# cure-lab/MagicDrive

Measured on NVIDIA H100. Metric: 6-view 224x400 denoising-steps/sec, higher is better.
Workload: dtype bf16

## Files before the change

include/magicdrive_b200.h:

```cpp
#ifndef MAGICDRIVE_B200_H
#define MAGICDRIVE_B200_H

#include <stddef.h>
#include <stdint.h>

#ifdef __cplusplus
extern "C" {
#endif

#define MDB_OK 0
#define MDB_ERR_INVALID (-1)
#define MDB_ERR_CUDA (-2)
#define MDB_ERR_UNSUPPORTED (-3)

const char* mdb_last_error(void);

int mdb_set_pdl(int on);
int mdb_version(void);
int mdb_device_ok(void);

typedef struct {
  const void* a0;
  const void* a1;
  int c0, lda0, c1, lda1;
  int n_img, h_in, w_in;
  const void* w;
  int n_out;
  int taps_h, taps_w, stride, pad_h, pad_w;
  int h_out, w_out;
  const float* bias;
  const float* rowbias;
  int rowbias_ld;
  const void* residual;
  int ldr;
  void* out;
  int ldo;
  int out_is_f32;
  float out_scale;
  int epi_mode;
  void* workspace;
  size_t workspace_bytes;
  int force_block_n;
  int force_splits;
  int kernel_variant;
  const float* ln_stats;
  int ln_parts;
  float ln_eps;
  const float* ln_colsum;
  float* stats_out;
} mdb_gemm_desc;

int mdb_gemm_conv(const mdb_gemm_desc* d, void* stream);
int mdb_gemm_conv_launches(const mdb_gemm_desc* d);
int mdb_gemm_conv_stats_parts(const mdb_gemm_desc* d);

int mdb_conv_direct(const void* x, int x_is_f32, int n, int h, int w, int cin, const float* wgt, const float* bias,
                    int cout, int kh, int kw, int stride_h, int stride_w, int pad_h, int pad_w, int ho, int wo,
                    int silu, const void* residual, void* out, int out_is_f32, void* stream);

int mdb_groupnorm(const void* x0, int c0, int ld0, const void* x1, int c1, int ld1, int n_img, int hw, int groups,
                  float eps, const float* gamma, const float* beta, int silu, void* out, int ldo, float* stats_ws,
                  void* stream);

int mdb_layernorm(const void* x, long long rows, int c, int ldx, const float* gamma, const float* beta, float eps,
                  void* out, int ldo, void* stream);

int mdb_softmax_rows(const float* s, int lds, long long rows, int cols, void* out, int ldo, int cols_out, void* stream);

int mdb_attention(const void* q, int ldq, const void* k, int ldk, const void* v, int ldv, void* out, int ldo, int b,
                  int b_kv, int heads, int lq, int lk, int d, const int* kv_index, int n_sets, float scale, void* stream);

int mdb_attention_multi(const void* q, int ldq, int n_src, const void* const* k, const int* ldk, const void* const* v,
                        const int* ldv, const int* b_kv, void* out, int ldo, int b, int heads, int lq, int lk, int d,
                        const int* kv_index, int n_sets, float scale, void* stream);

int mdb_add(const void* a, const void* b, void* out, long long n, void* stream);

int mdb_upsample_nearest(const void* x, int n, int h, int w, int c, void* out, int ho, int wo, void* stream);
int mdb_adaptive_avgpool(const float* x, int n, int h, int w, int c, float* out, int ho, int wo, int silu, void* stream);

int mdb_linear_small(const float* in, int m, int k, int ldi, const void* w, int ldw, const float* bias, int n,
                     int pre_silu, int post_silu, float* out, int ldo, void* stream);

int mdb_timestep_embedding(const float* t, int m, int dim, int flip_sin_to_cos, float freq_shift, float* out,
                           void* stream);

int mdb_fourier_embed(const float* x, long long rows, int d, int num_freqs, float* out, void* stream);
// ... 30 lines not shown
```

magicdrive_b200/_lib.py:

```python
import ctypes as C
import os
from pathlib import Path

_LIB = None
LIB_PATH = Path(os.environ.get("MDB_LIB_PATH") or Path(__file__).resolve().parent / "lib" / "libmagicdrive_b200.so")


class MdbError(RuntimeError):
    pass


class GemmDesc(C.Structure):
    _fields_ = [
        ("a0", C.c_void_p), ("a1", C.c_void_p),
        ("c0", C.c_int), ("lda0", C.c_int), ("c1", C.c_int), ("lda1", C.c_int),
        ("n_img", C.c_int), ("h_in", C.c_int), ("w_in", C.c_int),
        ("w", C.c_void_p), ("n_out", C.c_int),
        ("taps_h", C.c_int), ("taps_w", C.c_int), ("stride", C.c_int), ("pad_h", C.c_int), ("pad_w", C.c_int),
        ("h_out", C.c_int), ("w_out", C.c_int),
        ("bias", C.c_void_p), ("rowbias", C.c_void_p), ("rowbias_ld", C.c_int),
        ("residual", C.c_void_p), ("ldr", C.c_int),
        ("out", C.c_void_p), ("ldo", C.c_int), ("out_is_f32", C.c_int), ("out_scale", C.c_float),
        ("epi_mode", C.c_int),
        ("workspace", C.c_void_p), ("workspace_bytes", C.c_size_t),
        ("force_block_n", C.c_int), ("force_splits", C.c_int), ("kernel_variant", C.c_int),
        ("ln_stats", C.c_void_p), ("ln_parts", C.c_int), ("ln_eps", C.c_float), ("ln_colsum", C.c_void_p),
        ("stats_out", C.c_void_p),
    ]


_vp, _i, _f, _ll = C.c_void_p, C.c_int, C.c_float, C.c_longlong
SIGNATURES = {
    "mdb_last_error": (C.c_char_p, []),
    "mdb_set_pdl": (_i, [_i]),
    "mdb_version": (_i, []),
    "mdb_device_ok": (_i, []),
    "mdb_gemm_conv": (_i, [C.POINTER(GemmDesc), _vp]),
    "mdb_gemm_conv_launches": (_i, [C.POINTER(GemmDesc)]),
    "mdb_gemm_conv_stats_parts": (_i, [C.POINTER(GemmDesc)]),
    "mdb_conv_direct": (_i, [_vp, _i, _i, _i, _i, _i, _vp, _vp, _i, _i, _i, _i, _i, _i, _i, _i, _i, _i, _vp, _vp, _i, _vp]),
    "mdb_groupnorm": (_i, [_vp, _i, _i, _vp, _i, _i, _i, _i, _i, _f, _vp, _vp, _i, _vp, _i, _vp, _vp]),
    "mdb_layernorm": (_i, [_vp, _ll, _i, _i, _vp, _vp, _f, _vp, _i, _vp]),
    "mdb_attention": (_i, [_vp, _i, _vp, _i, _vp, _i, _vp, _i, _i, _i, _i, _i, _i, _i, _vp, _i, _f, _vp]),
    "mdb_attention_multi": (_i, [_vp, _i, _i, _vp, _vp, _vp, _vp, _vp, _vp, _i, _i, _i, _i, _i, _i, _vp, _i, _f, _vp]),
    "mdb_add": (_i, [_vp, _vp, _vp, _ll, _vp]),
    "mdb_upsample_nearest": (_i, [_vp, _i, _i, _i, _i, _vp, _i, _i, _vp]),
    "mdb_adaptive_avgpool": (_i, [_vp, _i, _i, _i, _i, _vp, _i, _i, _i, _vp]),
    "mdb_linear_small": (_i, [_vp, _i, _i, _i, _vp, _i, _vp, _i, _i, _i, _vp, _i, _vp]),
    "mdb_timestep_embedding": (_i, [_vp, _i, _i, _i, _f, _vp, _vp]),
    "mdb_fourier_embed": (_i, [_vp, _ll, _i, _i, _vp, _vp]),
    "mdb_nchw_to_nhwc": (_i, [_vp, _i, _i, _i, _i, _i, _vp, _vp]),
    "mdb_nhwc_to_nchw": (_i, [_vp, _i, _i, _i, _i, _vp, _i, _vp]),
    "mdb_f32_to_bf16": (_i, [_vp, _vp, _ll, _vp]),
    "mdb_bf16_to_f32": (_i, [_vp, _vp, _ll, _vp]),
    "mdb_pack_latents": (_i, [_vp, _i, _ll, _i, _i, _i, _vp, _vp]),
    "mdb_cfg_ddim_step": (_i, [_vp, _i, _i, _i, _f, _vp, _vp, _ll, _vp]),
    "mdb_softmax_rows": (_i, [_vp, _i, _ll, _i, _vp, _i, _i, _vp]),
    "mdb_pin_views": (_i, [_vp, _i, _vp, _vp, _i, _vp, _vp, _ll, _i, _vp]),
    "mdb_peer_barrier": (_i, [_vp, _i, _i, _i, _i, _vp, _ll, _vp, _vp]),
    "mdb_prepare_boxes": (_i, [_vp, _i, _vp, _vp, _i, _vp, _vp, _i, _i, _vp, _vp, _vp, _vp, _vp]),
    "mdb_camera_param": (_i, [_vp, _vp, _i, _vp, _vp]),
    "mdb_cfg_unipc_step": (_i, [_vp, _i, _i, _i, _f, _vp, _vp, _vp, _vp, _vp, _ll, _vp]),
}


def lib():
    global _LIB
    if _LIB is None:
        if not LIB_PATH.exists():
            raise MdbError(
                f"{LIB_PATH} is missing: build it with `python -m magicdrive_b200.build` "
                "(there is no CPU / torch fallback for this path)")
# ... 14 lines not shown
```

magicdrive_b200/csrc/capi_gemm.cu:

```cuda
#include <cuda.h>
#include <cuda_runtime.h>
#include <stdio.h>
#include <string.h>

#include <algorithm>
#include <mutex>

#include "../../include/magicdrive_b200.h"
#define MDB_NEED_TENSORMAP
#include "common_host.h"
#include "gemm_wgmma.cuh"

using namespace mdb;

namespace {

bool make_act_map(CUtensorMap* m, const void* ptr, int c, int ld, int n, int h, int w, int bn, int bh, int bw,
                  int stride) {
  EncodeTiledFn enc = get_encode();
  if (!enc) return false;
  cuuint64_t dims[4] = {(cuuint64_t)c, (cuuint64_t)w, (cuuint64_t)h, (cuuint64_t)n};
  cuuint64_t strides[3] = {(cuuint64_t)ld * 2, (cuuint64_t)w * ld * 2, (cuuint64_t)h * w * ld * 2};
  cuuint32_t box[4] = {64u, (cuuint32_t)(bw * stride), (cuuint32_t)(bh * stride), (cuuint32_t)bn};
  cuuint32_t estr[4] = {1u, (cuuint32_t)stride, (cuuint32_t)stride, 1u};
  CUresult r = enc(m, CU_TENSOR_MAP_DATA_TYPE_BFLOAT16, 4, const_cast<void*>(ptr), dims, strides, box, estr,
                   CU_TENSOR_MAP_INTERLEAVE_NONE, CU_TENSOR_MAP_SWIZZLE_128B, CU_TENSOR_MAP_L2_PROMOTION_L2_256B,
                   CU_TENSOR_MAP_FLOAT_OOB_FILL_NONE);
  return r == CUDA_SUCCESS;
}

bool make_w_map(CUtensorMap* m, const void* ptr, int n_out, int k, int block_n) {
  EncodeTiledFn enc = get_encode();
  if (!enc) return false;
  cuuint64_t dims[2] = {(cuuint64_t)k, (cuuint64_t)n_out};
  cuuint64_t strides[1] = {(cuuint64_t)k * 2};
  cuuint32_t box[2] = {64u, (cuuint32_t)block_n};
  cuuint32_t estr[2] = {1u, 1u};
  CUresult r = enc(m, CU_TENSOR_MAP_DATA_TYPE_BFLOAT16, 2, const_cast<void*>(ptr), dims, strides, box, estr,
                   CU_TENSOR_MAP_INTERLEAVE_NONE, CU_TENSOR_MAP_SWIZZLE_128B, CU_TENSOR_MAP_L2_PROMOTION_L2_256B,
                   CU_TENSOR_MAP_FLOAT_OOB_FILL_NONE);
  return r == CUDA_SUCCESS;
}

struct Plan {
  int bn, bh, bw, tiles_n, tiles_h, tiles_w;
  int ctas, m_groups;
  int block_n, n_tiles, splits, kb_per_split, kb_total;
};

int num_sms() {
  static int sms = 0;
  if (!sms) {
    int dev = 0;
    cudaGetDevice(&dev);
    if (cudaDeviceGetAttribute(&sms, cudaDevAttrMultiProcessorCount, dev) != cudaSuccess || sms <= 0) sms = 132;
  }
  return sms;
}

void choose_box(int n_img, int h, int w, Plan* pl) {
  if (h * w <= 128) {
    int bn = 128 / (h * w);
    if (bn > n_img) bn = n_img;
    if (bn < 1) bn = 1;
    pl->bn = bn, pl->bh = h, pl->bw = w;
  } else {
    double best = -1.0;
    int bbh = 1, bbw = 1;
    const int wmax = w < 128 ? w : 128;
    for (int bw = 1; bw <= wmax; ++bw) {
      int bh = 128 / bw;
      if (bh > h) bh = h;
      if (bh < 1) continue;
      const long long tiles = (long long)((h + bh - 1) / bh) * ((w + bw - 1) / bw);
      const double eff = (double)h * w / (double)(tiles * 128);
      if (eff > best + 1e-9 || (eff > best - 1e-9 && bw > bbw)) best = eff, bbh = bh, bbw = bw;
    }
    pl->bn = 1, pl->bh = bbh, pl->bw = bbw;
  }
  pl->tiles_n = (n_img + pl->bn - 1) / pl->bn;
  pl->tiles_h = (h + pl->bh - 1) / pl->bh;
  pl->tiles_w = (w + pl->bw - 1) / pl->bw;
}

int validate(const mdb_gemm_desc* d) {
  if (!d || !d->a0 || !d->w || !d->out) return set_error(MDB_ERR_INVALID, "mdb_gemm_conv: null pointer");
  if (d->c0 <= 0 || d->c0 % 64 || d->c1 < 0 || d->c1 % 64)
    return set_error(MDB_ERR_UNSUPPORTED, "mdb_gemm_conv: channel counts must be multiples of 64 (c0=%d c1=%d)", d->c0,
                     d->c1);
  if (d->c1 > 0 && !d->a1) return set_error(MDB_ERR_INVALID, "mdb_gemm_conv: c1>0 but a1 is null");
  if (d->lda0 % 8 || (d->c1 > 0 && d->lda1 % 8) || d->ldo % 8 || (d->residual && d->ldr % 8))
    return set_error(MDB_ERR_UNSUPPORTED, "mdb_gemm_conv: leading dimensions must be multiples of 8");
  if (d->n_out % 8) return set_error(MDB_ERR_UNSUPPORTED, "mdb_gemm_conv: n_out must be a multiple of 8");
  if (d->stride != 1 && d->stride != 2) return set_error(MDB_ERR_UNSUPPORTED, "mdb_gemm_conv: stride must be 1 or 2");
  if (d->kernel_variant != 0 && (d->kernel_variant < 2 || d->kernel_variant > 4))
    return set_error(MDB_ERR_INVALID, "mdb_gemm_conv: kernel_variant must be 0, 2, 3 or 4");
  if (d->n_img <= 0 || d->h_out <= 0 || d->w_out <= 0 || d->taps_h <= 0 || d->taps_w <= 0)
    return set_error(MDB_ERR_INVALID, "mdb_gemm_conv: bad shape");
  if ((reinterpret_cast<uintptr_t>(d->a0) | reinterpret_cast<uintptr_t>(d->a1) | reinterpret_cast<uintptr_t>(d->w) |
       reinterpret_cast<uintptr_t>(d->out) | reinterpret_cast<uintptr_t>(d->residual)) & 15)
    return set_error(MDB_ERR_INVALID, "mdb_gemm_conv: pointers must be 16-byte aligned");
  if (d->epi_mode == 1 && (d->n_out % 256 || d->residual || d->rowbias || d->out_is_f32 || d->stats_out))
    return set_error(MDB_ERR_UNSUPPORTED, "mdb_gemm_conv: GEGLU epilogue needs n_out %% 256 == 0 and a plain bf16 output "
                                          "(no residual, per-image shift or row statistics)");
  return MDB_OK;
}

void plan_for(const mdb_gemm_desc* d, int ctas, bool allow_split, Plan* pl) {
  choose_box(d->n_img, d->h_out, d->w_out, pl);
  const int m_tiles = pl->tiles_n * pl->tiles_h * pl->tiles_w;
  pl->ctas = ctas;
  pl->m_groups = (m_tiles + ctas - 1) / ctas;
  pl->kb_total = d->taps_h * d->taps_w * ((d->c0 + d->c1) / 64);
  const int sms = num_sms();
  const int clusters = sms / ctas;
  int bn_choice = 0;
  if (d->epi_mode == 1) {
    bn_choice = 256;
  } else if (d->force_block_n) {
    bn_choice = d->force_block_n;
  } else {
    const int cands[4] = {256, 160, 128, 64};
    double best = 1e30;
    for (int i = 0; i < 4; ++i) {
      const int bn = cands[i];
      if (bn == 64 && d->n_out >= 128) continue;
      const int nt = (d->n_out + bn - 1) / bn;
      const long long groups = (long long)pl->m_groups * nt;
      const long long waves = (groups + clusters - 1) / clusters;
      const double cost = (double)waves * (bn < 96 ? 96 : bn) * 1.0 + (double)waves * 6.0;
      if (cost < best - 1e-9) best = cost, bn_choice = bn;
    }
  }
  pl->block_n = bn_choice;
  pl->n_tiles = (d->n_out + bn_choice - 1) / bn_choice;
  int splits = 1;
  const long long ctas_total = (long long)m_tiles * pl->n_tiles;
  if (!allow_split) {
    splits = 1;
  } else if (d->force_splits > 0) {
    splits = d->force_splits;
  } else if (d->epi_mode == 0 && !d->ln_stats && !d->stats_out && d->workspace && ctas_total * 2 <= sms && pl->kb_total >= 16) {
    splits = (int)(sms / ctas_total);
// ... 42 lines not shown
  if (e == cudaSuccess) e = cudaGetLastError();
  if (e != cudaSuccess) return set_error(MDB_ERR_CUDA, "gemm_wgmma_kernel<%d,%d> launch: %s", BN, CTAS, cudaGetErrorString(e));
  return MDB_OK;
}

template <int CTAS>
int launch_bn(int block_n, const CUtensorMap& tA0, const CUtensorMap& tA1, const CUtensorMap& tB, const GemmParams& gp,
              cudaStream_t st) {
  switch (block_n) {
    case 256: return launch<256, CTAS>(tA0, tA1, tB, gp, st);
    case 160: return launch<160, CTAS>(tA0, tA1, tB, gp, st);
    case 128: return launch<128, CTAS>(tA0, tA1, tB, gp, st);
    case 64: return launch<64, CTAS>(tA0, tA1, tB, gp, st);
    default: return set_error(MDB_ERR_UNSUPPORTED, "mdb_gemm_conv: unsupported block_n %d", block_n);
  }
}

}

extern "C" int mdb_gemm_conv_launches(const mdb_gemm_desc* d) {
  if (validate(d) != MDB_OK) return MDB_ERR_INVALID;
  Plan pl;
  make_plan(d, &pl);
  return pl.splits > 1 ? 2 : 1;
}

extern "C" int mdb_gemm_conv_stats_parts(const mdb_gemm_desc* d) {
  if (validate(d) != MDB_OK) return MDB_ERR_INVALID;
  Plan pl;
  make_plan(d, &pl);
  return pl.n_tiles;
}

extern "C" int mdb_gemm_conv(const mdb_gemm_desc* d, void* stream) {
  int rc = validate(d);
  if (rc != MDB_OK) return rc;
  if (d->ln_stats && (d->taps_h != 1 || d->taps_w != 1 || !d->ln_colsum || d->ln_parts <= 0))
    return set_error(MDB_ERR_INVALID, "mdb_gemm_conv: a folded LayerNorm needs a 1x1 GEMM, ln_colsum and ln_parts");
  Plan pl;
  make_plan(d, &pl);
  if (d->epi_mode == 1 && pl.block_n != 256) return set_error(MDB_ERR_UNSUPPORTED, "GEGLU needs block_n 256");
  cudaStream_t st = static_cast<cudaStream_t>(stream);

  CUtensorMap tA0, tA1, tB;
  if (!make_act_map(&tA0, d->a0, d->c0, d->lda0, d->n_img, d->h_in, d->w_in, pl.bn, pl.bh, pl.bw, d->stride))
    return set_error(MDB_ERR_CUDA, "cuTensorMapEncodeTiled(A0) failed (c=%d ld=%d n=%d h=%d w=%d box=%dx%dx%d s=%d)",
                     d->c0, d->lda0, d->n_img, d->h_in, d->w_in, pl.bn, pl.bh, pl.bw, d->stride);
  if (d->c1 > 0) {
    if (!make_act_map(&tA1, d->a1, d->c1, d->lda1, d->n_img, d->h_in, d->w_in, pl.bn, pl.bh, pl.bw, d->stride))
      return set_error(MDB_ERR_CUDA, "cuTensorMapEncodeTiled(A1) failed");
  } else {
    tA1 = tA0;
  }
  const int ktot = d->taps_h * d->taps_w * (d->c0 + d->c1);
  if (!make_w_map(&tB, d->w, d->n_out, ktot, pl.block_n / pl.ctas))
    return set_error(MDB_ERR_CUDA, "cuTensorMapEncodeTiled(W) failed (n=%d k=%d)", d->n_out, ktot);

  GemmParams gp;
  memset(&gp, 0, sizeof(gp));
  gp.n_img = d->n_img, gp.h_out = d->h_out, gp.w_out = d->w_out, gp.n_out = d->n_out;
  gp.taps_h = d->taps_h, gp.taps_w = d->taps_w, gp.stride = d->stride, gp.pad_h = d->pad_h, gp.pad_w = d->pad_w;
  gp.cblocks0 = d->c0 / 64, gp.cblocks1 = d->c1 / 64;
  gp.bn = pl.bn, gp.bh = pl.bh, gp.bw = pl.bw, gp.tiles_h = pl.tiles_h, gp.tiles_w = pl.tiles_w;
  gp.m_tiles = pl.tiles_n * pl.tiles_h * pl.tiles_w, gp.n_tiles = pl.n_tiles, gp.splits = pl.splits;
  gp.m_groups = pl.m_groups;
  gp.kb_per_split = pl.kb_per_split;
  gp.epi_mode = pl.splits > 1 ? EPI_PARTIAL_F32 : d->epi_mode;
  gp.out_is_f32 = d->out_is_f32;
  gp.bias = d->bias, gp.rowbias = d->rowbias, gp.rowbias_ld = d->rowbias_ld;
  gp.residual = static_cast<const __nv_bfloat16*>(d->residual), gp.ldr = d->ldr;
  gp.out = d->out, gp.ldo = d->ldo, gp.out_scale = d->out_scale;
  gp.partial = static_cast<float*>(d->workspace);
  gp.ln_stats = d->ln_stats, gp.ln_parts = d->ln_parts, gp.ln_eps = d->ln_eps, gp.ln_colsum = d->ln_colsum;
  gp.ln_inv_c = 1.0f / (float)(d->c0 + d->c1);
  gp.stats_out = d->stats_out;

  rc = pl.ctas == 2 ? launch_bn<2>(pl.block_n, tA0, tA1, tB, gp, st) : launch_bn<1>(pl.block_n, tA0, tA1, tB, gp, st);
  if (rc != MDB_OK) return rc;
  if (pl.splits > 1) {
    const long long pixels = (long long)d->n_img * d->h_out * d->w_out;
    const long long total4 = pixels * d->n_out / 4;
    const int threads = 256;
    const int blocks = (int)((total4 + threads - 1) / threads);
    cudaError_t e = launch_pdl(splitk_finalize_kernel, dim3(blocks), dim3(threads), 0, st,
                               static_cast<const float*>(d->workspace), pl.splits, pixels, d->n_out, d->h_out * d->w_out,
                               d->bias, d->rowbias, d->rowbias_ld, static_cast<const __nv_bfloat16*>(d->residual), d->ldr,
                               d->out, d->ldo, d->out_is_f32, d->out_scale);
    if (e == cudaSuccess) e = cudaGetLastError();
    if (e != cudaSuccess) return set_error(MDB_ERR_CUDA, "splitk_finalize launch: %s", cudaGetErrorString(e));
  }
  return MDB_OK;
}
```

magicdrive_b200/csrc/common_host.h:

```cpp
#pragma once
#include <stdarg.h>
#include <stdio.h>

namespace mdb {
char* error_buffer();
inline int set_error(int code, const char* fmt, ...) {
  va_list ap;
  va_start(ap, fmt);
  vsnprintf(error_buffer(), 512, fmt, ap);
  va_end(ap);
  return code;
}
}

#ifdef MDB_NEED_TENSORMAP
#include <cuda.h>
#include <cuda_runtime.h>

#include <mutex>
namespace mdb {
typedef CUresult (*EncodeTiledFn)(CUtensorMap*, CUtensorMapDataType, cuuint32_t, void*, const cuuint64_t*,
                                  const cuuint64_t*, const cuuint32_t*, const cuuint32_t*, CUtensorMapInterleave,
                                  CUtensorMapSwizzle, CUtensorMapL2promotion, CUtensorMapFloatOOBfill);
inline EncodeTiledFn get_encode() {
  static EncodeTiledFn fn = nullptr;
  static std::once_flag once;
  std::call_once(once, [] {
    void* p = nullptr;
    cudaDriverEntryPointQueryResult qres;
    if (cudaGetDriverEntryPoint("cuTensorMapEncodeTiled", &p, cudaEnableDefault, &qres) == cudaSuccess &&
        qres == cudaDriverEntryPointSuccess)
      fn = reinterpret_cast<EncodeTiledFn>(p);
  });
  return fn;
}
}
#endif

#ifdef __CUDACC__
#include <cuda_runtime.h>
#include <stdlib.h>
namespace mdb {
inline int& pdl_region_flag() {
  static int v = 0;
  return v;
}
inline bool pdl_enabled() {
  static int forced = -2;
  if (forced == -2) {
    const char* e = getenv("MDB_PDL");
    forced = e ? ((e[0] == '1') ? 1 : 0) : -1;
  }
  return forced >= 0 ? forced == 1 : pdl_region_flag() == 1;
}
inline void add_pdl_attr(cudaLaunchConfig_t& cfg, cudaLaunchAttribute* attrs, unsigned n_attrs) {
  if (pdl_enabled()) {
    attrs[n_attrs].id = cudaLaunchAttributeProgrammaticStreamSerialization;
    attrs[n_attrs].val.programmaticStreamSerializationAllowed = 1;
    ++n_attrs;
  }
  cfg.attrs = attrs;
  cfg.numAttrs = n_attrs;
}
template <typename... KArgs, typename... Args>
inline cudaError_t launch_pdl(void (*kernel)(KArgs...), dim3 grid, dim3 block, size_t smem, cudaStream_t st, Args... args) {
// ... 23 lines not shown
```

magicdrive_b200/csrc/gemm_tc.cuh:

```cuda
#pragma once
#include "ptx.cuh"

namespace mdb {

enum EpiMode : int { EPI_LINEAR = 0, EPI_GEGLU = 1, EPI_PARTIAL_F32 = 2 };

struct GemmParams {
  int n_img, h_out, w_out;
  int n_out;
  int taps_h, taps_w, stride, pad_h, pad_w;
  int cblocks0, cblocks1;
  int bn, bh, bw;
  int tiles_h, tiles_w;
  int m_tiles, n_tiles, splits;
  int m_groups;
  int kb_per_split;
  int epi_mode;
  int out_is_f32;
  const float* bias;
  const float* rowbias;
  int rowbias_ld;
  const __nv_bfloat16* residual;
  int ldr;
  void* out;
  int ldo;
  float out_scale;
  float* partial;
  const float* ln_stats;
  int ln_parts;
  float ln_inv_c, ln_eps;
  const float* ln_colsum;
  float* stats_out;
};

constexpr int kBlockM = 128;
constexpr int kBlockK = 64;
constexpr int kABytes = kBlockM * kBlockK * 2;

__device__ __forceinline__ float gelu_erf(float x) {
  const float ax = fabsf(x) * 0.70710678118654752440f;
  float t, e;
  asm("rcp.approx.ftz.f32 %0, %1;" : "=f"(t) : "f"(fmaf(0.3275911f, ax, 1.0f)));
  float poly = fmaf(t, 1.061405429f, -1.453152027f);
  poly = fmaf(poly, t, 1.421413741f);
  poly = fmaf(poly, t, -0.284496736f);
  poly = fmaf(poly, t, 0.254829592f);
// ... 42 lines not shown
```

magicdrive_b200/csrc/gemm_wgmma.cuh:

```cuda
#pragma once
#include "common_host.h"
#include "gemm_tc.cuh"
#include "ptx_cluster.cuh"
#include "wgmma.cuh"

namespace mdb {

template <int BLOCK_N, int CTAS>
struct WgGemmCfg {
  static constexpr int kBBytes = BLOCK_N * kBlockK * 2;
  static constexpr int kBRows = BLOCK_N / CTAS;
  static constexpr int kBPartBytes = kBRows * kBlockK * 2;
  static constexpr int kStageBytes = kABytes + kBBytes;
  static constexpr int kBarBytes = 256;
  static constexpr int kStagesFit = (232448 - 1024 - kBarBytes) / kStageBytes;
  static constexpr int kStages = kStagesFit > 8 ? 8 : kStagesFit;
  static constexpr int kSmemBytes = kStages * kStageBytes + 1024 + kBarBytes;
  static constexpr int kConsumerWarps = 8;
  static constexpr int kThreads = 32 * kConsumerWarps + 32;
  static constexpr int kAcc = BLOCK_N / 2;
  static_assert(kStages >= 3, "pipeline too shallow");
  static_assert(kBPartBytes % 1024 == 0, "B stage parts must keep the 1024-byte swizzle alignment");
};

// ... 7 lines not shown
  constexpr bool PAIR = CTAS == 2;
  constexpr int STAGES = Cfg::kStages;
  extern __shared__ uint8_t smem_raw[];
  uint8_t* smem = reinterpret_cast<uint8_t*>((reinterpret_cast<uintptr_t>(smem_raw) + 1023) & ~uintptr_t(1023));
  uint8_t* smA = smem;
  uint8_t* smB = smem + STAGES * kABytes;
  uint64_t* full_bar = reinterpret_cast<uint64_t*>(smem + STAGES * Cfg::kStageBytes);
  uint64_t* empty_bar = full_bar + STAGES;

  const int warp = threadIdx.x >> 5;
  const int lane = threadIdx.x & 31;
  const int cb_total = p.cblocks0 + p.cblocks1;
  const int kb_total = p.taps_h * p.taps_w * cb_total;
  const int total_tiles = p.m_groups * p.n_tiles * p.splits;
  const int rank = PAIR ? static_cast<int>(cluster_ctarank()) : 0;
  const int first_tile = static_cast<int>(blockIdx.x) / CTAS, tile_step = static_cast<int>(gridDim.x) / CTAS;

  if (warp == Cfg::kConsumerWarps && lane == 0) {
    prefetch_tmap(&tmA0);
    prefetch_tmap(&tmA1);
    prefetch_tmap(&tmB);
    for (int i = 0; i < STAGES; ++i) {
      mbar_init(&full_bar[i], 1);
      mbar_init(&empty_bar[i], CTAS * Cfg::kConsumerWarps);
    }
    fence_barrier_init();
  }
  if constexpr (PAIR) cluster_sync_all(); else __syncthreads();
  pdl_wait();
  pdl_launch_dependents();

  if (warp == Cfg::kConsumerWarps) {
    if (lane == 0) {
      const uint32_t tx_bytes = static_cast<uint32_t>(p.bn * p.bh * p.bw) * (kBlockK * 2) + Cfg::kBBytes;
      int stage = 0;
      uint32_t phase = 0;
      for (int t = first_tile; t < total_tiles; t += tile_step) {
        const int mt = (t % p.m_groups) * CTAS + rank;
        const int rest = t / p.m_groups;
        const int nt = rest % p.n_tiles;
        const int z = rest / p.n_tiles;
        const int tw = mt % p.tiles_w;
        const int th = (mt / p.tiles_w) % p.tiles_h;
        const int tn = mt / (p.tiles_w * p.tiles_h);
        const int img0 = tn * p.bn, h0 = th * p.bh, w0 = tw * p.bw;
        const int n0 = nt * BLOCK_N;
        const int kb_begin = z * p.kb_per_split;
        const int kb_end = min(kb_total, kb_begin + p.kb_per_split);
        for (int kb = kb_begin; kb < kb_end; ++kb) {
          mbar_wait(&empty_bar[stage], phase ^ 1);
          const int tap = kb / cb_total;
          const int cb = kb - tap * cb_total;
          const int r = tap / p.taps_w, s = tap - r * p.taps_w;
          mbar_arrive_expect_tx(&full_bar[stage], tx_bytes);
          const int wc = w0 * p.stride + s - p.pad_w;
          const int hc = h0 * p.stride + r - p.pad_h;
          if (cb < p.cblocks0)
            tma_load_4d(&tmA0, &full_bar[stage], smA + stage * kABytes, cb * kBlockK, wc, hc, img0);
          else
            tma_load_4d(&tmA1, &full_bar[stage], smA + stage * kABytes, (cb - p.cblocks0) * kBlockK, wc, hc, img0);
          if constexpr (PAIR)
            tma_load_2d_multicast(&tmB, &full_bar[stage], smB + stage * Cfg::kBBytes + rank * Cfg::kBPartBytes, kb * kBlockK,
                                  n0 + rank * Cfg::kBRows, 0x3);
          else
            tma_load_2d(&tmB, &full_bar[stage], smB + stage * Cfg::kBBytes, kb * kBlockK, n0);
          if (++stage == STAGES) {
            stage = 0;
            phase ^= 1;
          }
        }
      }
    }
  } else {
  const int wg = warp >> 2;
  const int q = lane & 3;
  const int row0 = 64 * wg + 16 * (warp & 3) + (lane >> 2);
  const int box_hw = p.bh * p.bw;
  int li[2], lh[2], lw[2];
#pragma unroll
  for (int h = 0; h < 2; ++h) {
    const int row = row0 + 8 * h;
    li[h] = row / box_hw;
    const int rem = row - li[h] * box_hw;
    lh[h] = rem / p.bw;
    lw[h] = rem - lh[h] * p.bw;
  }
  const long long pixels_total = static_cast<long long>(p.n_img) * p.h_out * p.w_out;
  const float scale = p.out_scale;
  int stage = 0;
  uint32_t phase = 0;
  const uint32_t peer = rank ^ 1;
  auto release = [&](int s) {
    if (lane == 0) {
      mbar_arrive(&empty_bar[s]);
      if constexpr (PAIR) mbar_arrive_cluster_release(mapa_u32(smem_u32(&empty_bar[s]), peer));
    }
  };
  for (int t = first_tile; t < total_tiles; t += tile_step) {
    const int mt = (t % p.m_groups) * CTAS + rank;
    const int rest = t / p.m_groups;
    const int nt = rest % p.n_tiles;
    const int z = rest / p.n_tiles;
    const int tw = mt % p.tiles_w;
    const int th = (mt / p.tiles_w) % p.tiles_h;
    const int tn = mt / (p.tiles_w * p.tiles_h);
    const int n0 = nt * BLOCK_N;
    const int kb_begin = z * p.kb_per_split;
    const int nkb = min(kb_total, kb_begin + p.kb_per_split) - kb_begin;

    float acc[Cfg::kAcc];
#pragma unroll
    for (int i = 0; i < Cfg::kAcc; ++i) acc[i] = 0.f;
    int prev = -1;
    for (int i = 0; i < nkb; ++i) {
      mbar_wait(&full_bar[stage], phase);
      wgmma_fence();
      const uint64_t adesc = make_sw128_kmajor_desc(smem_u32(smA + stage * kABytes + wg * (64 * 128)));
      const uint64_t bdesc = make_sw128_kmajor_desc(smem_u32(smB + stage * Cfg::kBBytes));
#pragma unroll
      for (int k = 0; k < kBlockK / 16; ++k) WgmmaSS<BLOCK_N>::run(acc, adesc + 2 * k, bdesc + 2 * k, 1u);
      wgmma_commit();
      wgmma_wait<1>();
      if (prev >= 0) release(prev);
      prev = stage;
      if (++stage == STAGES) {
        stage = 0;
        phase ^= 1;
      }
    }
    wgmma_wait<0>();
    if (prev >= 0) release(prev);

    int img[2];
    long long pix[2];
    bool ok[2];
#pragma unroll
    for (int h = 0; h < 2; ++h) {
      img[h] = tn * p.bn + li[h];
      const int oh = th * p.bh + lh[h], ow = tw * p.bw + lw[h];
      ok[h] = (li[h] < p.bn) && (img[h] < p.n_img) && (oh < p.h_out) && (ow < p.w_out);
      pix[h] = (static_cast<long long>(img[h]) * p.h_out + oh) * p.w_out + ow;
    }
    if (p.epi_mode == EPI_PARTIAL_F32) {
#pragma unroll
      for (int j = 0; j < BLOCK_N / 8; ++j) {
        const int col = n0 + 8 * j + 2 * q;
        if (col >= p.n_out) continue;
#pragma unroll
        for (int h = 0; h < 2; ++h)
          if (ok[h])
            *reinterpret_cast<float2*>(p.partial + (static_cast<long long>(z) * pixels_total + pix[h]) * p.n_out + col) =
                make_float2(acc[4 * j + 2 * h], acc[4 * j + 2 * h + 1]);
      }
      continue;
    }
    float rowA[2] = {scale, scale}, rowB[2] = {0.f, 0.f};
    if (p.ln_stats != nullptr) {
#pragma unroll
      for (int h = 0; h < 2; ++h) {
        if (!ok[h]) continue;
        const float2* sp = reinterpret_cast<const float2*>(p.ln_stats) + pix[h] * p.ln_parts;
        float s = 0.f, ss = 0.f;
        for (int j = 0; j < p.ln_parts; ++j) {
          const float2 v = __ldg(sp + j);
          s += v.x, ss += v.y;
        }
        const float mean = s * p.ln_inv_c;
        const float rstd = rsqrtf(fmaxf(ss * p.ln_inv_c - mean * mean, 0.f) + p.ln_eps);
        rowA[h] = rstd * scale;
        rowB[h] = -mean * rowA[h];
      }
    }
    const bool has_ln = p.ln_stats != nullptr;
    if (p.epi_mode == EPI_GEGLU) {
// ... 70 lines not shown
```

magicdrive_b200/csrc/ptx.cuh:

```cuda
#pragma once
#include <cuda.h>
#include <cuda_bf16.h>
#include <cuda_runtime.h>
#include <stdint.h>

namespace mdb {

__device__ __forceinline__ uint32_t smem_u32(const void* p) {
  return static_cast<uint32_t>(__cvta_generic_to_shared(p));
}

__device__ __forceinline__ bool elect_one() {
  uint32_t pred = 0;
  asm volatile(
      "{\n\t"
      ".reg .pred P;\n\t"
      "elect.sync _|P, 0xffffffff;\n\t"
      "selp.b32 %0, 1, 0, P;\n\t"
      "}\n"
      : "=r"(pred));
  return pred != 0;
}

__device__ __forceinline__ void mbar_init(uint64_t* bar, uint32_t count) {
// ... 56 lines not shown
#else
  asm volatile(
      "{\n\t"
      ".reg .pred P1;\n\t"
      "WAIT_LOOP:\n\t"
      "mbarrier.test_wait.parity.shared::cta.b64 P1, [%0], %1;\n\t"
      "@P1 bra DONE;\n\t"
      "bra WAIT_LOOP;\n\t"
      "DONE:\n\t"
      "}\n" ::"r"(smem_u32(bar)),
      "r"(parity)
      : "memory");
#endif
}

__device__ __forceinline__ void prefetch_tmap(const CUtensorMap* m) {
  asm volatile("prefetch.tensormap [%0];" ::"l"(reinterpret_cast<uint64_t>(m)) : "memory");
}
__device__ __forceinline__ void tma_load_2d(const CUtensorMap* m, uint64_t* bar, void* dst, int c0, int c1) {
  asm volatile(
      "cp.async.bulk.tensor.2d.shared::cluster.global.mbarrier::complete_tx::bytes"
      " [%0], [%1, {%3, %4}], [%2];" ::"r"(smem_u32(dst)),
      "l"(reinterpret_cast<uint64_t>(m)), "r"(smem_u32(bar)), "r"(c0), "r"(c1)
      : "memory");
}
__device__ __forceinline__ void tma_load_4d(const CUtensorMap* m, uint64_t* bar, void* dst, int c0, int c1, int c2,
                                            int c3) {
  asm volatile(
      "cp.async.bulk.tensor.4d.shared::cluster.global.mbarrier::complete_tx::bytes"
      " [%0], [%1, {%3, %4, %5, %6}], [%2];" ::"r"(smem_u32(dst)),
      "l"(reinterpret_cast<uint64_t>(m)), "r"(smem_u32(bar)), "r"(c0), "r"(c1), "r"(c2), "r"(c3)
      : "memory");
}

__device__ __forceinline__ uint64_t make_sw128_kmajor_desc(uint32_t smem_addr_bytes) {
  uint64_t d = 0;
  d |= static_cast<uint64_t>((smem_addr_bytes >> 4) & 0x3FFF);
  d |= static_cast<uint64_t>(1) << 16;
  d |= static_cast<uint64_t>((1024u >> 4) & 0x3FFF) << 32;
  d |= static_cast<uint64_t>(1) << 62;
  return d;
}
__device__ __forceinline__ uint64_t make_sw128_mnmajor_desc(uint32_t smem_addr_bytes, uint32_t lbo_bytes) {
  uint64_t d = 0;
  d |= static_cast<uint64_t>((smem_addr_bytes >> 4) & 0x3FFF);
  d |= static_cast<uint64_t>((lbo_bytes >> 4) & 0x3FFF) << 16;
  d |= static_cast<uint64_t>((1024u >> 4) & 0x3FFF) << 32;
  d |= static_cast<uint64_t>(1) << 62;
  return d;
}

__device__ __forceinline__ uint32_t pack_bf16(float a, float b) {
  __nv_bfloat162 h = __floats2bfloat162_rn(a, b);
  return *reinterpret_cast<uint32_t*>(&h);
}

}
```

magicdrive_b200/ops.py:

```python
import ctypes as C
import contextlib
import os
from typing import Optional

import torch

from . import _lib
from ._lib import GemmDesc, check

BF16 = torch.bfloat16
F32 = torch.float32

GEMM_VARIANT = int(os.environ.get('MDB_GEMM_VARIANT', '0'))
_launches = 0
_profile = None


def start_profile():
    global _profile
    _profile = []


def stop_profile(with_info: bool = False):
    global _profile
# ... 103 lines not shown
    d.a0, d.a1 = _ptr(a0), _ptr(a1)
    d.c0, d.lda0, d.c1, d.lda1 = c0, lda0, c1, lda1
    d.n_img, d.h_in, d.w_in = n_img, h_in, w_in
    d.w, d.n_out = _ptr(w), n_out
    d.taps_h = d.taps_w = taps
    d.stride, d.pad_h, d.pad_w = stride, pad, pad
    d.h_out, d.w_out = h_out, w_out
    d.bias = _ptr(bias)
    d.rowbias = _ptr(rowbias)
    d.rowbias_ld = (rowbias.stride(0) if rowbias.shape[0] > 1 else 0) if rowbias is not None else 0
    d.residual, d.ldr = _ptr(residual), ldr
    d.out, d.ldo, d.out_is_f32, d.out_scale = _ptr(out), ldo, int(out_f32), float(out_scale)
    d.epi_mode = 1 if geglu else 0
    if allow_split_k and not geglu:
        ws = workspace(64 << 20, a0.device)
        d.workspace, d.workspace_bytes = ws.data_ptr(), ws.numel()
    else:
        d.workspace, d.workspace_bytes = None, 0
    d.force_block_n, d.force_splits = force_block_n, force_splits
    d.kernel_variant = kernel_variant or GEMM_VARIANT
    L = _lib.lib()
    if ln is not None:
        d.ln_stats, d.ln_parts, d.ln_eps, d.ln_colsum = ln.data.data_ptr(), ln.parts, float(ln_eps), _ptr(ln_colsum)
    stats = None
    if emit_stats:
        d.stats_out = 1
        parts = L.mdb_gemm_conv_stats_parts(C.byref(d))
        if parts <= 0:
            check(parts, "mdb_gemm_conv_stats_parts")
        stats = RowStats(torch.empty((pixels, parts, 2), dtype=F32, device=a0.device), parts)
        d.stats_out = stats.data.data_ptr()
    e0 = _prof_begin()
    check(L.mdb_gemm_conv(C.byref(d), _stream()), "mdb_gemm_conv")
    _prof_end("gemm_conv", 2.0 * pixels * n_out * taps * taps * (c0 + c1), e0,
              f"M={pixels} N={n_out} K={taps * taps * (c0 + c1)} img={n_img}x{h_out}x{w_out} taps={taps} s={stride} "
              f"geglu={int(geglu)} res={int(residual is not None)}")
    _launches += L.mdb_gemm_conv_launches(C.byref(d))
    return (out, stats) if emit_stats else out


@contextlib.contextmanager
def pdl_region(enabled: bool = True):
    lib = _lib.lib()
    old = lib.mdb_set_pdl(int(enabled))
    try:
        yield
    finally:
        lib.mdb_set_pdl(old)


def linear(x: torch.Tensor, w: torch.Tensor, bias=None, residual=None, out=None, ldo=None, geglu=False,
           out_f32=False, out_scale=1.0, **kw):
    m, k = x.shape
    return gemm_conv(x, w, n_img=1, h_in=1, w_in=m, c0=k, lda0=x.stride(0), n_out=w.shape[0], bias=bias,
                     residual=residual, ldr=(residual.stride(0) if residual is not None else 0), out=out, ldo=ldo,
                     geglu=geglu, out_f32=out_f32, out_scale=out_scale, **kw)


def conv_direct(x, wgt, bias, *, n, h, w, cin, cout, k, stride=(1, 1), pad=(1, 1), silu=False, residual=None,
                out_f32=False):
    global _launches
    _need_cuda(x, wgt)
    ho = (h + 2 * pad[0] - k) // stride[0] + 1
    wo = (w + 2 * pad[1] - k) // stride[1] + 1
    out = torch.empty((n, ho, wo, cout), dtype=F32 if out_f32 else BF16, device=x.device)
    check(_lib.lib().mdb_conv_direct(_ptr(x), int(x.dtype == F32), n, h, w, cin, _ptr(wgt), _ptr(bias), cout, k, k,
                                     stride[0], stride[1], pad[0], pad[1], ho, wo, int(silu), _ptr(residual),
                                     _ptr(out), int(out_f32), _stream()), "mdb_conv_direct")
    _launches += 1
# ... 205 lines not shown
```

Baseline: 54.07.

## Use TMA im2col loads and flat pixel M-tiles for conv GEMM

Replaces the 4D tiled activation box (chosen per image shape with bn/bh/bw) with flat 128-pixel M tiles. Convolutions now use TMA im2col-mode tensor maps with per-tap offsets, and 1x1 or linear cases use a plain 2D row map. This removes padding waste from partial spatial boxes on awkward shapes like 28x50 and simplifies the epilogue's pixel indexing. A profiling-only plan query is also added. The risk is im2col TMA behaviour at image boundaries and some per-tile address arithmetic in the producer.

After: 56.64, median of 6. 4.8% higher.

```diff
diff --git a/include/magicdrive_b200.h b/include/magicdrive_b200.h
--- a/include/magicdrive_b200.h
+++ b/include/magicdrive_b200.h
@@ -53,6 +53,7 @@
 int mdb_gemm_conv(const mdb_gemm_desc* d, void* stream);
 int mdb_gemm_conv_launches(const mdb_gemm_desc* d);
 int mdb_gemm_conv_stats_parts(const mdb_gemm_desc* d);
+int mdb_gemm_conv_plan(const mdb_gemm_desc* d, int* plan);
 
 int mdb_conv_direct(const void* x, int x_is_f32, int n, int h, int w, int cin, const float* wgt, const float* bias,
                     int cout, int kh, int kw, int stride_h, int stride_w, int pad_h, int pad_w, int ho, int wo,
diff --git a/magicdrive_b200/_lib.py b/magicdrive_b200/_lib.py
--- a/magicdrive_b200/_lib.py
+++ b/magicdrive_b200/_lib.py
@@ -38,6 +38,7 @@
     "mdb_gemm_conv": (_i, [C.POINTER(GemmDesc), _vp]),
     "mdb_gemm_conv_launches": (_i, [C.POINTER(GemmDesc)]),
     "mdb_gemm_conv_stats_parts": (_i, [C.POINTER(GemmDesc)]),
+    "mdb_gemm_conv_plan": (_i, [C.POINTER(GemmDesc), C.POINTER(C.c_int)]),
     "mdb_conv_direct": (_i, [_vp, _i, _i, _i, _i, _i, _vp, _vp, _i, _i, _i, _i, _i, _i, _i, _i, _i, _i, _vp, _vp, _i, _vp]),
     "mdb_groupnorm": (_i, [_vp, _i, _i, _vp, _i, _i, _i, _i, _i, _f, _vp, _vp, _i, _vp, _i, _vp, _vp]),
     "mdb_layernorm": (_i, [_vp, _ll, _i, _i, _vp, _vp, _f, _vp, _i, _vp]),
diff --git a/magicdrive_b200/csrc/capi_gemm.cu b/magicdrive_b200/csrc/capi_gemm.cu
--- a/magicdrive_b200/csrc/capi_gemm.cu
+++ b/magicdrive_b200/csrc/capi_gemm.cu
@@ -15,18 +15,37 @@
 
 namespace {
 
-bool make_act_map(CUtensorMap* m, const void* ptr, int c, int ld, int n, int h, int w, int bn, int bh, int bw,
-                  int stride) {
+bool make_im2col_map(CUtensorMap* m, const void* ptr, int c, int ld, const mdb_gemm_desc* d) {
+  EncodeIm2colFn enc = get_encode_im2col();
+  if (!enc) return false;
+  const int n = d->n_img, h = d->h_in, w = d->w_in;
+  cuuint64_t dims[4] = {(cuuint64_t)c, (cuuint64_t)w, (cuuint64_t)h, (cuuint64_t)n};
+  cuuint64_t strides[3] = {(cuuint64_t)ld * 2, (cuuint64_t)w * ld * 2, (cuuint64_t)h * w * ld * 2};
+  int lower[2] = {-d->pad_w, -d->pad_h};
+  int upper[2] = {d->pad_w - (d->taps_w - 1), d->pad_h - (d->taps_h - 1)};
+  cuuint32_t estr[4] = {1u, (cuuint32_t)d->stride, (cuuint32_t)d->stride, 1u};
+  CUresult r = enc(m, CU_TENSOR_MAP_DATA_TYPE_BFLOAT16, 4, const_cast<void*>(ptr), dims, strides, lower, upper, 64u,
+                   (cuuint32_t)kBlockM, estr, CU_TENSOR_MAP_INTERLEAVE_NONE, CU_TENSOR_MAP_SWIZZLE_128B,
+                   CU_TENSOR_MAP_L2_PROMOTION_L2_256B, CU_TENSOR_MAP_FLOAT_OOB_FILL_NONE);
+  return r == CUDA_SUCCESS;
+}
+
+bool make_rows_map(CUtensorMap* m, const void* ptr, int c, int ld, long long pixels) {
   EncodeTiledFn enc = get_encode();
   if (!enc) return false;
-  cuuint64_t dims[4] = {(cuuint64_t)c, (cuuint64_t)w, (cuuint64_t)h, (cuuint64_t)n};
-  cuuint64_t strides[3] = {(cuuint64_t)ld * 2, (cuuint64_t)w * ld * 2, (cuuint64_t)h * w * ld * 2};
-  cuuint32_t box[4] = {64u, (cuuint32_t)(bw * stride), (cuuint32_t)(bh * stride), (cuuint32_t)bn};
-  cuuint32_t estr[4] = {1u, (cuuint32_t)stride, (cuuint32_t)stride, 1u};
-  CUresult r = enc(m, CU_TENSOR_MAP_DATA_TYPE_BFLOAT16, 4, const_cast<void*>(ptr), dims, strides, box, estr,
+  cuuint64_t dims[2] = {(cuuint64_t)c, (cuuint64_t)pixels};
+  cuuint64_t strides[1] = {(cuuint64_t)ld * 2};
+  cuuint32_t box[2] = {64u, (cuuint32_t)kBlockM};
+  cuuint32_t estr[2] = {1u, 1u};
+  CUresult r = enc(m, CU_TENSOR_MAP_DATA_TYPE_BFLOAT16, 2, const_cast<void*>(ptr), dims, strides, box, estr,
                    CU_TENSOR_MAP_INTERLEAVE_NONE, CU_TENSOR_MAP_SWIZZLE_128B, CU_TENSOR_MAP_L2_PROMOTION_L2_256B,
                    CU_TENSOR_MAP_FLOAT_OOB_FILL_NONE);
   return r == CUDA_SUCCESS;
+}
+
+bool make_act_map(CUtensorMap* m, const void* ptr, int c, int ld, const mdb_gemm_desc* d, bool im2col) {
+  return im2col ? make_im2col_map(m, ptr, c, ld, d)
+                : make_rows_map(m, ptr, c, ld, (long long)d->n_img * d->h_out * d->w_out);
 }
 
 bool make_w_map(CUtensorMap* m, const void* ptr, int n_out, int k, int block_n) {
@@ -43,7 +62,7 @@
 }
 
 struct Plan {
-  int bn, bh, bw, tiles_n, tiles_h, tiles_w;
+  int m_tiles;
   int ctas, m_groups;
   int block_n, n_tiles, splits, kb_per_split, kb_total;
 };
@@ -56,31 +75,6 @@
     if (cudaDeviceGetAttribute(&sms, cudaDevAttrMultiProcessorCount, dev) != cudaSuccess || sms <= 0) sms = 132;
   }
   return sms;
-}
-
-void choose_box(int n_img, int h, int w, Plan* pl) {
-  if (h * w <= 128) {
-    int bn = 128 / (h * w);
-    if (bn > n_img) bn = n_img;
-    if (bn < 1) bn = 1;
-    pl->bn = bn, pl->bh = h, pl->bw = w;
-  } else {
-    double best = -1.0;
-    int bbh = 1, bbw = 1;
-    const int wmax = w < 128 ? w : 128;
-    for (int bw = 1; bw <= wmax; ++bw) {
-      int bh = 128 / bw;
-      if (bh > h) bh = h;
-      if (bh < 1) continue;
-      const long long tiles = (long long)((h + bh - 1) / bh) * ((w + bw - 1) / bw);
-      const double eff = (double)h * w / (double)(tiles * 128);
-      if (eff > best + 1e-9 || (eff > best - 1e-9 && bw > bbw)) best = eff, bbh = bh, bbw = bw;
-    }
-    pl->bn = 1, pl->bh = bbh, pl->bw = bbw;
-  }
-  pl->tiles_n = (n_img + pl->bn - 1) / pl->bn;
-  pl->tiles_h = (h + pl->bh - 1) / pl->bh;
-  pl->tiles_w = (w + pl->bw - 1) / pl->bw;
 }
 
 int validate(const mdb_gemm_desc* d) {
@@ -107,8 +101,8 @@
 }
 
 void plan_for(const mdb_gemm_desc* d, int ctas, bool allow_split, Plan* pl) {
-  choose_box(d->n_img, d->h_out, d->w_out, pl);
-  const int m_tiles = pl->tiles_n * pl->tiles_h * pl->tiles_w;
+  const int m_tiles = (int)(((long long)d->n_img * d->h_out * d->w_out + kBlockM - 1) / kBlockM);
+  pl->m_tiles = m_tiles;
   pl->ctas = ctas;
   pl->m_groups = (m_tiles + ctas - 1) / ctas;
   pl->kb_total = d->taps_h * d->taps_w * ((d->c0 + d->c1) / 64);
@@ -217,6 +211,20 @@
   return pl.n_tiles;
 }
 
+extern "C" int mdb_gemm_conv_plan(const mdb_gemm_desc* d, int* plan) {
+  if (validate(d) != MDB_OK) return MDB_ERR_INVALID;
+  Plan pl;
+  make_plan(d, &pl);
+  const long long walk = (long long)pl.m_groups * pl.n_tiles * pl.splits;
+  const int clusters = num_sms() / pl.ctas;
+  plan[0] = pl.block_n;
+  plan[1] = pl.m_tiles;
+  plan[2] = pl.n_tiles;
+  plan[3] = pl.splits;
+  plan[4] = (int)((walk + clusters - 1) / clusters);
+  return MDB_OK;
+}
+
 extern "C" int mdb_gemm_conv(const mdb_gemm_desc* d, void* stream) {
   int rc = validate(d);
   if (rc != MDB_OK) return rc;
@@ -227,13 +235,16 @@
   if (d->epi_mode == 1 && pl.block_n != 256) return set_error(MDB_ERR_UNSUPPORTED, "GEGLU needs block_n 256");
   cudaStream_t st = static_cast<cudaStream_t>(stream);
 
+  const bool im2col = d->taps_h != 1 || d->taps_w != 1 || d->stride != 1 || d->pad_h || d->pad_w ||
+                      d->h_in != d->h_out || d->w_in != d->w_out;
   CUtensorMap tA0, tA1, tB;
-  if (!make_act_map(&tA0, d->a0, d->c0, d->lda0, d->n_img, d->h_in, d->w_in, pl.bn, pl.bh, pl.bw, d->stride))
-    return set_error(MDB_ERR_CUDA, "cuTensorMapEncodeTiled(A0) failed (c=%d ld=%d n=%d h=%d w=%d box=%dx%dx%d s=%d)",
-                     d->c0, d->lda0, d->n_img, d->h_in, d->w_in, pl.bn, pl.bh, pl.bw, d->stride);
+  if (!make_act_map(&tA0, d->a0, d->c0, d->lda0, d, im2col))
+    return set_error(MDB_ERR_CUDA, "cuTensorMapEncode%s(A0) failed (c=%d ld=%d n=%d h=%d w=%d taps=%dx%d pad=%dx%d s=%d)",
+                     im2col ? "Im2col" : "Tiled", d->c0, d->lda0, d->n_img, d->h_in, d->w_in, d->taps_h, d->taps_w,
+                     d->pad_h, d->pad_w, d->stride);
   if (d->c1 > 0) {
-    if (!make_act_map(&tA1, d->a1, d->c1, d->lda1, d->n_img, d->h_in, d->w_in, pl.bn, pl.bh, pl.bw, d->stride))
-      return set_error(MDB_ERR_CUDA, "cuTensorMapEncodeTiled(A1) failed");
+    if (!make_act_map(&tA1, d->a1, d->c1, d->lda1, d, im2col))
+      return set_error(MDB_ERR_CUDA, "cuTensorMapEncode%s(A1) failed", im2col ? "Im2col" : "Tiled");
   } else {
     tA1 = tA0;
   }
@@ -246,8 +257,8 @@
   gp.n_img = d->n_img, gp.h_out = d->h_out, gp.w_out = d->w_out, gp.n_out = d->n_out;
   gp.taps_h = d->taps_h, gp.taps_w = d->taps_w, gp.stride = d->stride, gp.pad_h = d->pad_h, gp.pad_w = d->pad_w;
   gp.cblocks0 = d->c0 / 64, gp.cblocks1 = d->c1 / 64;
-  gp.bn = pl.bn, gp.bh = pl.bh, gp.bw = pl.bw, gp.tiles_h = pl.tiles_h, gp.tiles_w = pl.tiles_w;
-  gp.m_tiles = pl.tiles_n * pl.tiles_h * pl.tiles_w, gp.n_tiles = pl.n_tiles, gp.splits = pl.splits;
+  gp.im2col = im2col;
+  gp.m_tiles = pl.m_tiles, gp.n_tiles = pl.n_tiles, gp.splits = pl.splits;
   gp.m_groups = pl.m_groups;
   gp.kb_per_split = pl.kb_per_split;
   gp.epi_mode = pl.splits > 1 ? EPI_PARTIAL_F32 : d->epi_mode;
diff --git a/magicdrive_b200/csrc/common_host.h b/magicdrive_b200/csrc/common_host.h
--- a/magicdrive_b200/csrc/common_host.h
+++ b/magicdrive_b200/csrc/common_host.h
@@ -31,6 +31,22 @@
     if (cudaGetDriverEntryPoint("cuTensorMapEncodeTiled", &p, cudaEnableDefault, &qres) == cudaSuccess &&
         qres == cudaDriverEntryPointSuccess)
       fn = reinterpret_cast<EncodeTiledFn>(p);
+  });
+  return fn;
+}
+typedef CUresult (*EncodeIm2colFn)(CUtensorMap*, CUtensorMapDataType, cuuint32_t, void*, const cuuint64_t*,
+                                   const cuuint64_t*, const int*, const int*, cuuint32_t, cuuint32_t, const cuuint32_t*,
+                                   CUtensorMapInterleave, CUtensorMapSwizzle, CUtensorMapL2promotion,
+                                   CUtensorMapFloatOOBfill);
+inline EncodeIm2colFn get_encode_im2col() {
+  static EncodeIm2colFn fn = nullptr;
+  static std::once_flag once;
+  std::call_once(once, [] {
+    void* p = nullptr;
+    cudaDriverEntryPointQueryResult qres;
+    if (cudaGetDriverEntryPoint("cuTensorMapEncodeIm2col", &p, cudaEnableDefault, &qres) == cudaSuccess &&
+        qres == cudaDriverEntryPointSuccess)
+      fn = reinterpret_cast<EncodeIm2colFn>(p);
   });
   return fn;
 }
diff --git a/magicdrive_b200/csrc/gemm_tc.cuh b/magicdrive_b200/csrc/gemm_tc.cuh
--- a/magicdrive_b200/csrc/gemm_tc.cuh
+++ b/magicdrive_b200/csrc/gemm_tc.cuh
@@ -10,8 +10,7 @@
   int n_out;
   int taps_h, taps_w, stride, pad_h, pad_w;
   int cblocks0, cblocks1;
-  int bn, bh, bw;
-  int tiles_h, tiles_w;
+  int im2col;
   int m_tiles, n_tiles, splits;
   int m_groups;
   int kb_per_split;
diff --git a/magicdrive_b200/csrc/gemm_wgmma.cuh b/magicdrive_b200/csrc/gemm_wgmma.cuh
--- a/magicdrive_b200/csrc/gemm_wgmma.cuh
+++ b/magicdrive_b200/csrc/gemm_wgmma.cuh
@@ -63,7 +63,8 @@
 
   if (warp == Cfg::kConsumerWarps) {
     if (lane == 0) {
-      const uint32_t tx_bytes = static_cast<uint32_t>(p.bn * p.bh * p.bw) * (kBlockK * 2) + Cfg::kBBytes;
+      const uint32_t tx_bytes = kABytes + Cfg::kBBytes;
+      const int hw_out = p.h_out * p.w_out;
       int stage = 0;
       uint32_t phase = 0;
       for (int t = first_tile; t < total_tiles; t += tile_step) {
@@ -71,10 +72,11 @@
         const int rest = t / p.m_groups;
         const int nt = rest % p.n_tiles;
         const int z = rest / p.n_tiles;
-        const int tw = mt % p.tiles_w;
-        const int th = (mt / p.tiles_w) % p.tiles_h;
-        const int tn = mt / (p.tiles_w * p.tiles_h);
-        const int img0 = tn * p.bn, h0 = th * p.bh, w0 = tw * p.bw;
+        const int pix0 = mt * kBlockM;
+        const int img0 = pix0 / hw_out;
+        const int oh0 = (pix0 - img0 * hw_out) / p.w_out;
+        const int ow0 = pix0 - img0 * hw_out - oh0 * p.w_out;
+        const int wc = ow0 * p.stride - p.pad_w, hc = oh0 * p.stride - p.pad_h;
         const int n0 = nt * BLOCK_N;
         const int kb_begin = z * p.kb_per_split;
         const int kb_end = min(kb_total, kb_begin + p.kb_per_split);
@@ -84,12 +86,13 @@
           const int cb = kb - tap * cb_total;
           const int r = tap / p.taps_w, s = tap - r * p.taps_w;
           mbar_arrive_expect_tx(&full_bar[stage], tx_bytes);
-          const int wc = w0 * p.stride + s - p.pad_w;
-          const int hc = h0 * p.stride + r - p.pad_h;
-          if (cb < p.cblocks0)
-            tma_load_4d(&tmA0, &full_bar[stage], smA + stage * kABytes, cb * kBlockK, wc, hc, img0);
+          const CUtensorMap* tmA = cb < p.cblocks0 ? &tmA0 : &tmA1;
+          const int c = (cb < p.cblocks0 ? cb : cb - p.cblocks0) * kBlockK;
+          if (p.im2col)
+            tma_load_im2col_4d(tmA, &full_bar[stage], smA + stage * kABytes, c, wc, hc, img0, static_cast<uint16_t>(s),
+                               static_cast<uint16_t>(r));
           else
-            tma_load_4d(&tmA1, &full_bar[stage], smA + stage * kABytes, (cb - p.cblocks0) * kBlockK, wc, hc, img0);
+            tma_load_2d(tmA, &full_bar[stage], smA + stage * kABytes, c, pix0);
           if constexpr (PAIR)
             tma_load_2d_multicast(&tmB, &full_bar[stage], smB + stage * Cfg::kBBytes + rank * Cfg::kBPartBytes, kb * kBlockK,
                                   n0 + rank * Cfg::kBRows, 0x3);
@@ -106,16 +109,7 @@
   const int wg = warp >> 2;
   const int q = lane & 3;
   const int row0 = 64 * wg + 16 * (warp & 3) + (lane >> 2);
-  const int box_hw = p.bh * p.bw;
-  int li[2], lh[2], lw[2];
-#pragma unroll
-  for (int h = 0; h < 2; ++h) {
-    const int row = row0 + 8 * h;
-    li[h] = row / box_hw;
-    const int rem = row - li[h] * box_hw;
-    lh[h] = rem / p.bw;
-    lw[h] = rem - lh[h] * p.bw;
-  }
+  const int hw_out = p.h_out * p.w_out;
   const long long pixels_total = static_cast<long long>(p.n_img) * p.h_out * p.w_out;
   const float scale = p.out_scale;
   int stage = 0;
@@ -132,9 +126,6 @@
     const int rest = t / p.m_groups;
     const int nt = rest % p.n_tiles;
     const int z = rest / p.n_tiles;
-    const int tw = mt % p.tiles_w;
-    const int th = (mt / p.tiles_w) % p.tiles_h;
-    const int tn = mt / (p.tiles_w * p.tiles_h);
     const int n0 = nt * BLOCK_N;
     const int kb_begin = z * p.kb_per_split;
     const int nkb = min(kb_total, kb_begin + p.kb_per_split) - kb_begin;
@@ -167,10 +158,10 @@
     bool ok[2];
 #pragma unroll
     for (int h = 0; h < 2; ++h) {
-      img[h] = tn * p.bn + li[h];
-      const int oh = th * p.bh + lh[h], ow = tw * p.bw + lw[h];
-      ok[h] = (li[h] < p.bn) && (img[h] < p.n_img) && (oh < p.h_out) && (ow < p.w_out);
-      pix[h] = (static_cast<long long>(img[h]) * p.h_out + oh) * p.w_out + ow;
+      const int px = mt * kBlockM + row0 + 8 * h;
+      img[h] = px / hw_out;
+      pix[h] = px;
+      ok[h] = pix[h] < pixels_total;
     }
     if (p.epi_mode == EPI_PARTIAL_F32) {
 #pragma unroll
diff --git a/magicdrive_b200/csrc/ptx.cuh b/magicdrive_b200/csrc/ptx.cuh
--- a/magicdrive_b200/csrc/ptx.cuh
+++ b/magicdrive_b200/csrc/ptx.cuh
@@ -112,6 +112,14 @@
       "l"(reinterpret_cast<uint64_t>(m)), "r"(smem_u32(bar)), "r"(c0), "r"(c1), "r"(c2), "r"(c3)
       : "memory");
 }
+__device__ __forceinline__ void tma_load_im2col_4d(const CUtensorMap* m, uint64_t* bar, void* dst, int c, int w, int h,
+                                                   int n, uint16_t off_w, uint16_t off_h) {
+  asm volatile(
+      "cp.async.bulk.tensor.4d.shared::cluster.global.im2col.mbarrier::complete_tx::bytes"
+      " [%0], [%1, {%3, %4, %5, %6}], [%2], {%7, %8};" ::"r"(smem_u32(dst)),
+      "l"(reinterpret_cast<uint64_t>(m)), "r"(smem_u32(bar)), "r"(c), "r"(w), "r"(h), "r"(n), "h"(off_w), "h"(off_h)
+      : "memory");
+}
 
 __device__ __forceinline__ uint64_t make_sw128_kmajor_desc(uint32_t smem_addr_bytes) {
   uint64_t d = 0;
diff --git a/magicdrive_b200/ops.py b/magicdrive_b200/ops.py
--- a/magicdrive_b200/ops.py
+++ b/magicdrive_b200/ops.py
@@ -159,9 +159,13 @@
         d.stats_out = stats.data.data_ptr()
     e0 = _prof_begin()
     check(L.mdb_gemm_conv(C.byref(d), _stream()), "mdb_gemm_conv")
-    _prof_end("gemm_conv", 2.0 * pixels * n_out * taps * taps * (c0 + c1), e0,
-              f"M={pixels} N={n_out} K={taps * taps * (c0 + c1)} img={n_img}x{h_out}x{w_out} taps={taps} s={stride} "
-              f"geglu={int(geglu)} res={int(residual is not None)}")
+    if e0 is not None:
+        plan = (C.c_int * 5)()
+        check(L.mdb_gemm_conv_plan(C.byref(d), plan), "mdb_gemm_conv_plan")
+        _prof_end("gemm_conv", 2.0 * pixels * n_out * taps * taps * (c0 + c1), e0,
+                  f"M={pixels} N={n_out} K={taps * taps * (c0 + c1)} img={n_img}x{h_out}x{w_out} taps={taps} s={stride} "
+                  f"geglu={int(geglu)} res={int(residual is not None)} | BN={plan[0]} tiles={plan[1]}x{plan[2]}x{plan[3]} "
+                  f"waves={plan[4]}")
     _launches += L.mdb_gemm_conv_launches(C.byref(d))
     return (out, stats) if emit_stats else out
 
```
